# InfiniteNightmare/HNSW-Slim

Hardware: AMD Instinct MI355X
Metric: QPS @ recall@10>=0.95 (SIFT-1M d=128, k=10) (higher is better)
Workload: dtype f32

## Files before the change

### hnsw-slim_amd/csrc/flat_search.hip

```cpp
#include <hip/hip_runtime.h>

#include <algorithm>
#include <cfloat>
#include <climits>

#include "dist_recipe.hpp"
#include "engine.hpp"
#include "heap_emul.hpp"
#include "narrow_load.hpp"
#include "search_common.hpp"
#include "sorted_insert.hpp"
#include "wave_util.hpp"

namespace hs {

typedef __attribute__((address_space(3))) unsigned char lds_u8;
typedef __attribute__((address_space(3))) uint32_t lds_u32;
typedef __attribute__((address_space(3))) unsigned short lds_u16;
typedef uint32_t hs_u4 __attribute__((ext_vector_type(4)));
typedef __attribute__((address_space(3))) hs_u4 lds_u128;
typedef __attribute__((address_space(3))) float lds_f32;
typedef __attribute__((address_space(3))) hs_f2 lds_f2;
typedef unsigned short hs_us2 __attribute__((ext_vector_type(2)));

static constexpr uint32_t kFlatOvfCap = 64;
static constexpr uint32_t kFlatBucketTags = 7;

struct FlatLds { uint32_t off_q, off_vis, off_ovf, off_nid, total; };
__host__ __device__ inline FlatLds flat_layout(uint32_t dim, uint32_t ef, uint32_t nb) {
  FlatLds l;
  l.off_q = 0;
  l.off_vis = align_up(dim * 4, 16);
  const uint32_t vis_bytes = nb * 16 > (ef + 1) * 8 ? nb * 16 : (ef + 1) * 8;
  l.off_ovf = l.off_vis + align_up(vis_bytes, 16);
  l.off_nid = l.off_ovf + kFlatOvfCap * 4;
  l.total = l.off_nid + 64 * 4;
  return l;
}

__device__ __forceinline__ uint32_t pk_min_u16(uint32_t a, uint32_t b) {
  return __builtin_bit_cast(uint32_t, __builtin_elementwise_min(__builtin_bit_cast(hs_us2, a), __builtin_bit_cast(hs_us2, b)));
}
template <int METRIC>
__device__ __forceinline__ int dkey(float d) {
  const int b = (int)__float_as_uint(d);
  return METRIC == METRIC_L2 ? b : (b ^ ((b >> 31) & 0x7FFFFFFF));
}
template <int METRIC>
__device__ __forceinline__ float key_dist(int k) {
  return __uint_as_float((uint32_t)(METRIC == METRIC_L2 ? k : (k ^ ((k >> 31) & 0x7FFFFFFF))));
}
static constexpr int kFKeyInf = 0x7F800000;
static constexpr uint32_t kFDone = 0x80000000u;

__device__ __forceinline__ int wave_min_i32_f(int v) {
#define HS_SHR_MINI(ctrl) v = min(v, __builtin_amdgcn_update_dpp(INT_MAX, v, ctrl, 0xf, 0xf, false))
  HS_SHR_MINI(0x111); HS_SHR_MINI(0x112); HS_SHR_MINI(0x114); HS_SHR_MINI(0x118);
#undef HS_SHR_MINI
  const int r0 = __builtin_amdgcn_readlane(v, 15), r1 = __builtin_amdgcn_readlane(v, 31);
  const int r2 = __builtin_amdgcn_readlane(v, 47), r3 = __builtin_amdgcn_readlane(v, 63);
  return min(min(r0, r1), min(r2, r3));
}

__host__ __device__ constexpr int flat_row_buffer(int d16) {
#ifdef HS_FLAT_LONG_B
  return d16 <= 0 ? 1 : d16 <= 8 ? d16 : (d16 < HS_FLAT_LONG_B ? d16 : HS_FLAT_LONG_B);
#else
  return d16 <= 0 ? 1 : d16 <= 8 ? d16 : d16 % 30 == 0 ? 30 : d16 % 32 == 0 ? 32 : d16 % 24 == 0 ? 24 : 16;
#endif
}
__host__ __device__ constexpr int flat_waves(int s, int d16) {
#ifdef HS_FLAT_WAVES
  return HS_FLAT_WAVES;
#else
#ifdef HS_FLAT_LONG_WAVES
  return d16 > 8 ? HS_FLAT_LONG_WAVES : d16 < 0 ? 3 : s > 4 ? 4 : 5;
#else
  return d16 > 8 ? 2 : d16 < 0 ? 3 : s > 4 ? 4 : 5;
#endif
#endif
}


template <int METRIC, int D16, typename ROW>
__device__ __forceinline__ float flat_dist8(const ROW *vec, uint32_t dim, const lds_u8 *qv, uint32_t rowid, int s) {
  const lds_f2 *qq = reinterpret_cast<const lds_f2 *>(qv) + s;
  hs_f2 acc = {0.f, 0.f};
  auto step = [&](const hs_f2 q2, const hs_f2 x) {
    if (METRIC == METRIC_L2) {
      const hs_f2 t = q2 - x;
      const hs_f2 p = t * t;
      acc = acc + p;
    } else {
      acc = __builtin_elementwise_fma(q2, x, acc);
    }
  };
  if constexpr (RowKind<ROW>::narrow) {
    const ROW *chunk = vec + (size_t)rowid * dim + (uint32_t)s * (dim >> 3);
    if constexpr (D16 > 0) {
      constexpr int NDW = D16 * (int)sizeof(ROW) / 2;
      static_assert(D16 * sizeof(ROW) % 2 == 0, "a lane's chunk is a whole number of dwords");
      const uint32_t *cp = reinterpret_cast<const uint32_t *>(chunk);
      uint32_t dw[NDW];
#pragma unroll
      for (int j = 0; j + 4 <= NDW; j += 4) {
        const hs_u4_a4 v = *reinterpret_cast<const hs_u4_a4 *>(cp + j);
        dw[j] = v.x; dw[j + 1] = v.y; dw[j + 2] = v.z; dw[j + 3] = v.w;
      }
      if constexpr ((NDW & 2) != 0) {
        const hs_u2_a4 v = *reinterpret_cast<const hs_u2_a4 *>(cp + (NDW & ~3));
        dw[NDW & ~3] = v.x; dw[(NDW & ~3) + 1] = v.y;
      }
      if constexpr ((NDW & 1) != 0) dw[NDW - 1] = cp[NDW - 1];
#pragma unroll
      for (int i = 0; i < D16; i++) {
        if (D16 > 8 && i % 8 == 0) __builtin_amdgcn_sched_barrier(0);
        step(qq[i * 8], narrow_pair((const ROW *)nullptr, dw, i));
      }
    } else {
      constexpr uint32_t RB = D16 == 0 ? 8u : 16u;
      const uint32_t steps = dim >> 4;
      for (uint32_t r0 = 0; r0 < steps; r0 += RB) {
        const uint32_t nb = min(RB, steps - r0);
        hs_f2 buf[RB];
#pragma unroll
        for (uint32_t i = 0; i < RB; i++)
          if (i < nb) buf[i] = narrow_pair_at(chunk, r0 + i);
#pragma unroll
        for (uint32_t i = 0; i < RB; i++)
          if (i < nb) step(qq[(r0 + i) * 8], buf[i]);
      }
    }
  } else {
  const hs_f2 *row = reinterpret_cast<const hs_f2 *>(vec + (size_t)rowid * dim) + s;
  if (D16 > 0) {
    constexpr int B = flat_row_buffer(D16);
    constexpr int R = (D16 > 0 ? D16 : 1) / B, T = (D16 > 0 ? D16 : 1) % B;
    hs_f2 buf[B];
#pragma unroll
    for (int i = 0; i < B; i++) buf[i] = row[i * 8];
#pragma unroll
    for (int i = 0; i < B; i++) {
      if (B > 8 && i % 8 == 0) __builtin_amdgcn_sched_barrier(0);
      step(qq[i * 8], buf[i]);
    }
#pragma unroll 1
    for (int r = 1; r < R; r++) {
#pragma unroll
      for (int i = 0; i < B; i++) buf[i] = row[(r * B + i) * 8];
#pragma unroll
      for (int i = 0; i < B; i++) step(qq[(r * B + i) * 8], buf[i]);
    }
    if (T > 0) {
#pragma unroll
      for (int i = 0; i < T; i++) buf[i] = row[(R * B + i) * 8];
#pragma unroll
      for (int i = 0; i < T; i++) step(qq[(R * B + i) * 8], buf[i]);
    }
  } else {
    constexpr uint32_t RB = D16 == 0 ? 8u : 16u;
    const uint32_t steps = dim >> 4;
    for (uint32_t r0 = 0; r0 < steps; r0 += RB) {
      const uint32_t nb = min(RB, steps - r0);
      hs_f2 buf[RB];
#pragma unroll
      for (uint32_t i = 0; i < RB; i++)
        if (i < nb) buf[i] = row[(r0 + i) * 8];
#pragma unroll
      for (uint32_t i = 0; i < RB; i++)
        if (i < nb) step(qq[(r0 + i) * 8], buf[i]);
    }
  }
  }
  if (METRIC == METRIC_L2) {
    float r = acc.x + acc.y;
#pragma unroll
    for (int k = 1; k < 8; k++) {
      float t;
      asm("s_nop 1\n\tv_add_f32_dpp %0, %1, %2 row_shr:1 row_mask:0xf bank_mask:0xf" : "=v"(t) : "v"(r), "v"(acc.x));
      r = t + acc.y;
    }
    return r;
  } else {
    float hx = acc.x + dpp_f<0x104>(acc.x), hy = acc.y + dpp_f<0x104>(acc.y);
    hx = hx + dpp_f<0x102>(hx); hy = hy + dpp_f<0x102>(hy);
    hx = hx + dpp_f<0x101>(hx); hy = hy + dpp_f<0x101>(hy);
    return 1.0f - (hx + hy);
  }
}

struct FlatHeap {
  lds_u8 *lds;
  uint2 *glob;
  uint32_t L;
};
typedef uint32_t hs_u2 __attribute__((ext_vector_type(2)));
typedef __attribute__((address_space(3))) hs_u2 lds_u64;
template <bool T2>
__device__ __forceinline__ uint2 fh_get(const FlatHeap &h, uint32_t s) {
  if (!T2 || s < h.L) { const hs_u2 v = *reinterpret_cast<lds_u64 *>(h.lds + s * 8); return make_uint2(v.x, v.y); }
  return h.glob[s];
}
template <bool T2>
__device__ __forceinline__ void fh_set(const FlatHeap &h, uint32_t s, uint2 v) {
  if (!T2 || s < h.L) *reinterpret_cast<lds_u64 *>(h.lds + s * 8) = hs_u2{v.x, v.y};
  else h.glob[s] = v;
}
template <bool T2>
__device__ __forceinline__ uint4 fh_get2(const FlatHeap &h, uint32_t s ) {
  if (!T2 || s < h.L) { const hs_u4 v = *reinterpret_cast<lds_u128 *>(h.lds + s * 8); return make_uint4(v.x, v.y, v.z, v.w); }
  return *reinterpret_cast<const uint4 *>(&h.glob[s]);
}
template <bool T2>
__device__ __forceinline__ void fh_push(const FlatHeap &h, uint32_t n , float d, uint32_t id, int lane) {
  const uint32_t anc = n >> (lane + 1);
  const bool has = anc != 0 && lane < 31;
  uint2 p = make_uint2(0, 0);
  if (has) p = fh_get<T2>(h, anc);
  const unsigned long long rises = hs_ballot(has && __uint_as_float(p.x) > d);
  const uint32_t r = __ffsll((long long)~rises) - 1;
  if ((uint32_t)lane < r) fh_set<T2>(h, n >> lane, p);
  if ((uint32_t)lane == r) fh_set<T2>(h, n >> r, make_uint2(__float_as_uint(d), id));
}
template <bool T2>
__device__ __forceinline__ void fh_pop(const FlatHeap &h, uint32_t n ) {
  if (n <= 1) return;
  const uint2 v = fh_get<T2>(h, n);
  const uint32_t len = n - 1;
  uint32_t hole = 0, child = 0;
  while (child < (len - 1) / 2) {
    child = 2 * (child + 1);
    const uint4 two = fh_get2<T2>(h, child);
    const bool left = __uint_as_float(two.z) > __uint_as_float(two.x);
    fh_set<T2>(h, hole + 1, left ? make_uint2(two.x, two.y) : make_uint2(two.z, two.w));
    child = left ? child - 1 : child;
    hole = child;
  }
  if ((len & 1) == 0 && child == (len - 2) / 2) {
    child = 2 * (child + 1);
    fh_set<T2>(h, hole + 1, fh_get<T2>(h, child));
    hole = child - 1;
  }
  const float vd = __uint_as_float(v.x);
  while (hole > 0) {
    const uint32_t parent = (hole - 1) >> 1;
    const uint2 p = fh_get<T2>(h, parent + 1);
    if (!(__uint_as_float(p.x) > vd)) break;
    fh_set<T2>(h, hole + 1, p);
    hole = parent;
  }
  fh_set<T2>(h, hole + 1, v);
}

__device__ __forceinline__ void fh_pop_wave(const FlatHeap &h, uint32_t n , int lane) {
  if (n <= 1) return;
  const uint2 v = fh_get<false>(h, n);
  const uint32_t len = n - 1;
  uint32_t hole = 0;
  const uint32_t dl = lane < 1 ? 0u : (lane < 3 ? 1u : 2u);
  const uint32_t ol = (uint32_t)lane + 1u - (1u << dl);
  while (true) {
    const uint32_t node = ((hole + 1u) << dl) - 1u + ol;
    const bool two = lane < 7 && 2u * node + 2u < len;
    uint4 pr = make_uint4(0, 0, 0, 0);
    if (two) pr = fh_get2<false>(h, 2u * node + 2u);
    const bool right = !(__uint_as_float(pr.z) > __uint_as_float(pr.x));
    const unsigned long long vm = hs_ballot(two), rm = hs_ballot(two && right);
    uint32_t l = 0, path = 0, last = 0;
    bool open = true;
#pragma unroll
    for (int kk = 0; kk < 3; kk++) {
      const bool ok = open && ((vm >> l) & 1ull);
      if (ok) { path |= 1u << l; last = l; l = 2u * l + 1u + (uint32_t)((rm >> l) & 1ull); }
      open = ok;
    }
    if (path == 0) break;
    const uint32_t child = 2u * node + 1u + (right ? 1u : 0u);
    if (lane < 7 && ((path >> lane) & 1u)) fh_set<false>(h, node + 1u, right ? make_uint2(pr.z, pr.w) : make_uint2(pr.x, pr.y));
    hole = __builtin_amdgcn_readlane(child, last);
    if (!open) break;
  }
  if ((len & 1u) == 0 && hole == (len - 2u) / 2u) {
    const uint2 c = fh_get<false>(h, 2u * hole + 2u);
    if (lane == 0) fh_set<false>(h, hole + 1u, c);
    hole = 2u * hole + 1u;
  }
  wave_sync();
  fh_push<false>(h, hole + 1u, __uint_as_float(v.x), v.y, lane);
}

struct FlatSync {
  lds_u8 *vis;
  uint32_t *scratch;
  uint32_t heap_lds_slots, off_heap, off_log, off_hop, hop_cap, cand_total;
  uint32_t n_log, hop0, hl, lb_bits;
  uint32_t cand_size, hp, hq, h_idx;
};
struct FlatSyncOut { uint32_t cand_size, hp, hq, h_idx, rc, stop, next_id; };
#ifdef HS_FLAT_SYNC_CALL
#define HS_FLAT_SYNC_ATTR __attribute__((noinline))
#else
#define HS_FLAT_SYNC_ATTR __forceinline__
#endif
template <int METRIC>
__device__ HS_FLAT_SYNC_ATTR FlatSyncOut flat_heap_sync(FlatSync f) {
  const int lane = threadIdx.x;
  lds_u8 *vis = (lds_u8 *)(uintptr_t)uni((uint32_t)(uintptr_t)f.vis);
  const uint64_t sbits = (uint64_t)(uintptr_t)f.scratch;
  uint32_t *scratch = reinterpret_cast<uint32_t *>((uintptr_t)(((uint64_t)uni((uint32_t)(sbits >> 32)) << 32) | uni((uint32_t)sbits)));
  uint2 *heap_store = reinterpret_cast<uint2 *>(scratch + uni(f.off_heap));
  const uint2 *tlog = reinterpret_cast<const uint2 *>(scratch + uni(f.off_log));
  const uint32_t *hoplog = scratch + uni(f.off_hop);
  hs_u4 *park = reinterpret_cast<hs_u4 *>(scratch + uni(f.off_hop) + uni(f.hop_cap));
  const uint32_t heap_lds_slots = uni(f.heap_lds_slots), n_log = uni(f.n_log), hop0 = uni(f.hop0), hl = f.hl, cand_total = uni(f.cand_total);
  const int lb = (int)uni(f.lb_bits);
  uint32_t cand_size = uni(f.cand_size), hp = uni(f.hp), hq = uni(f.hq), h_idx = uni(f.h_idx), rc = 0, next_id = 0;
  __threadfence_block();
  for (uint32_t i = lane; i * 2u < heap_lds_slots; i += 64) park[i] = *reinterpret_cast<lds_u128 *>(vis + i * 16);
  FlatHeap cand;
  cand.lds = vis;
  cand.L = heap_lds_slots;
  cand.glob = heap_store;
  wave_sync();
  for (uint32_t sl = lane; sl <= cand_size && sl < heap_lds_slots; sl += 64) {
    const uint2 e = heap_store[sl];
    *reinterpret_cast<lds_u64 *>(vis + sl * 8) = hs_u2{e.x, e.y};
  }
  wave_sync();
  uint32_t ebase = ~0u;
  uint2 eb = make_uint2(0, 0);
  auto log_at = [&](uint32_t i) -> uint2 {
    if ((i & ~63u) != ebase) {
      ebase = i & ~63u;
      eb = (ebase + lane < n_log) ? tlog[ebase + lane] : make_uint2(0, 0);
    }
    return make_uint2(__builtin_amdgcn_readlane(eb.x, i & 63u), __builtin_amdgcn_readlane(eb.y, i & 63u));
  };
  if (h_idx == 0) {
    const uint2 e = log_at(0);
    cand_size = 1;
    fh_push<false>(cand, cand_size, __uint_as_float(e.x), e.y, lane);
    wave_sync();
    h_idx = 1;
  }
  const uint32_t ring_base = hop0 & ~63u;
  uint32_t hbase = ~0u, hcnt = 0;
  while (hq < hop0) {
    if (hp == hq) {
      if (cand_size < heap_lds_slots) fh_pop_wave(cand, cand_size, lane);
      else if (lane == 0) fh_pop<true>(cand, cand_size);
      cand_size--;
      hp++;
      wave_sync();
    }
    if ((hq & ~63u) != hbase) {
      hbase = hq & ~63u;
      hcnt = hbase == ring_base ? hl : hoplog[hbase + lane];
    }
    const uint32_t np = (uint32_t)__builtin_amdgcn_readlane(hcnt, hq & 63u);
    if (__builtin_expect(cand_size + np > cand_total, 0)) { rc = 2; break; }
    const bool in_lds = cand_size + np < heap_lds_slots;
    for (uint32_t q = 0; q < np; q++) {
      const uint2 e = log_at(h_idx);
      cand_size++;
      if (in_lds) fh_push<false>(cand, cand_size, __uint_as_float(e.x), e.y, lane);
      else fh_push<true>(cand, cand_size, __uint_as_float(e.x), e.y, lane);
      wave_sync();
      h_idx++;
    }
    hq++;
  }
  bool stop = rc != 0 || cand_size == 0;
  if (!stop) {
    const uint2 root = fh_get<false>(cand, 1);
    const uint32_t rkey_bits = uni(root.x);
    if (dkey<METRIC>(__uint_as_float(rkey_bits)) > lb) {
      stop = true;
    } else {
      next_id = uni(root.y);
      if (cand_size < heap_lds_slots) fh_pop_wave(cand, cand_size, lane);
      else if (lane == 0) fh_pop<true>(cand, cand_size);
      cand_size--;
      hp++;
      wave_sync();
    }
  }
  for (uint32_t sl = lane; sl <= cand_size && sl < heap_lds_slots; sl += 64) {
    const hs_u2 e = *reinterpret_cast<lds_u64 *>(vis + sl * 8);
    heap_store[sl] = make_uint2(e.x, e.y);
  }
  wave_sync();
  __threadfence_block();
  for (uint32_t i = lane; i * 2u < heap_lds_slots; i += 64) *reinterpret_cast<lds_u128 *>(vis + i * 16) = park[i];
  wave_sync();
  FlatSyncOut o;
  o.cand_size = cand_size; o.hp = hp; o.hq = hq; o.h_idx = h_idx; o.rc = rc; o.stop = stop ? 1u : 0u; o.next_id = next_id;
  return o;
}

template <int S>
__device__ __forceinline__ int rank_key(const int (&tk)[S], uint32_t r) {
  const uint32_t l = r / S, sl = r % S;
  int v = __builtin_amdgcn_readlane(tk[0], l);
#pragma unroll
  for (int s = 1; s < S; s++) {
    const int t = __builtin_amdgcn_readlane(tk[s], l);
    v = sl == (uint32_t)s ? t : v;
  }
  return v;
}

template <int METRIC, int S, int D16, typename ROW>
__device__ int search_one_flat(const DevIndex &ix, const SearchArgs &a, const uint32_t qi, lds_u8 *smem, const ROW *rows) {
  const int lane = threadIdx.x;
  constexpr int OWN = METRIC == METRIC_L2 ? 7 : 0;
  const int s8 = lane & 7, grp = lane >> 3;
  const uint32_t dim = D16 > 0 ? (uint32_t)D16 * 16u : ix.dim;
  const FlatLds L = flat_layout(dim, a.ef, a.fl_nb);
  lds_u8 *qv = smem + L.off_q;
  lds_u8 *vis = smem + L.off_vis;
  lds_u32 *ovf = reinterpret_cast<lds_u32 *>(smem + L.off_ovf);
  lds_u32 *nid = reinterpret_cast<lds_u32 *>(smem + L.off_nid);
  const uint32_t k = a.k, ef = a.ef;
  uint32_t *scratch = a.spill + (size_t)qi * a.spill_stride;
  uint2 *tlog = reinterpret_cast<uint2 *>(scratch + a.spill_slots + 2 * a.cand2_cap);
  uint32_t *hoplog = scratch + a.spill_slots + 2 * a.cand2_cap + 2 * a.log_cap;
  const uint32_t hop_cap = a.hop_cap / 4;
  uint32_t n_dist = 1, n_hops = 0, n_nbr = 0;
#ifdef HS_FLAT_DIAG
  const unsigned long long diag_t0 = __builtin_amdgcn_s_memrealtime();
  uint32_t diag_syncs = 0, diag_replayed = 0, diag_sync_ticks = 0, diag_pre = 0;
  uint32_t diag_ph[6] = {0, 0, 0, 0, 0, 0};
  unsigned long long diag_tp = __builtin_amdgcn_s_memtime();
#define HS_DIAG_LAP(i) { const unsigned long long t_ = __builtin_amdgcn_s_memtime(); diag_ph[i] += (uint32_t)(t_ - diag_tp); diag_tp = t_; }
#else
#define HS_DIAG_LAP(i)
#endif

  for (uint32_t i = lane; i < dim; i += 64) reinterpret_cast<lds_f32 *>(qv)[i] = a.queries[(size_t)qi * dim + i];
  for (uint32_t i = lane; i < a.fl_nb; i += 64) *reinterpret_cast<lds_u128 *>(vis + i * 16) = hs_u4{~0u, ~0u, ~0u, 0x0000FFFFu};
  uint32_t ovf_n = 0;
  const uint32_t vmask = a.vis_bits >= 32 ? 0xFFFFFFFFu : (1u << a.vis_bits) - 1u;
  const uint32_t nb = a.fl_nb, vmul = a.fl_mul, vsh = a.fl_sh;
  wave_sync();

  bool vfail = false;
  Visited v2;
  v2.t2 = scratch;
  v2.slots2 = a.spill_slots;
  v2.limit2 = a.spill_slots - (a.spill_slots >> 2);
  v2.n2 = 0;
  v2.spilled = false;
  auto vis_mark = [&](const uint32_t id, const bool valid) -> bool {
    const uint32_t h32 = id * 2654435761u;
    const uint32_t h = h32 & vmask;
    const uint32_t tag = __umulhi(h, vmul) >> vsh;
    const uint32_t b = h - tag * nb;
    lds_u8 *bp = vis + b * 16;
    const hs_u4 w = *reinterpret_cast<lds_u128 *>(bp);
    const uint32_t t2 = tag | (tag << 16);
    const uint32_t m = pk_min_u16(pk_min_u16(w.x ^ t2, w.y ^ t2), pk_min_u16(w.z ^ t2, (w.w ^ tag) | 0xFFFF0000u));
    const bool hit = (m & 0xFFFFu) == 0 || (m >> 16) == 0;
    bool isnew = valid && !hit;
    bool done = false;
    unsigned long long lm = hs_ballot(isnew && (w.w >> 16) >= kFlatBucketTags);
    if (__builtin_expect(lm != 0 && ovf_n != 0, 0)) {
      const uint32_t mine = (uint32_t)lane < ovf_n ? ovf[lane] : kNone;
      unsigned long long todo = lm;
      while (todo) {
        const int j = __ffsll((long long)todo) - 1;
        todo &= todo - 1;
        const uint32_t idj = __builtin_amdgcn_readlane(id, j);
        const bool found = hs_ballot(mine == idj) != 0;
        if (found && lane == j) isnew = false;
      }
      if (v2.spilled) {
        const bool mine2 = isnew && ((lm >> lane) & 1ull);
        if (mine2) { isnew = vis_insert_t2(v2, id, h32); done = true; }
        v2.n2 += __popcll(hs_ballot(mine2 && isnew));
      }
    }
    uint32_t e = 0;
    if (isnew && !done) {
      const uint32_t old = __hip_atomic_fetch_add(reinterpret_cast<lds_u32 *>(bp + 12), 0x10000u, __ATOMIC_RELAXED, __HIP_MEMORY_SCOPE_WAVEFRONT);
      e = old >> 16;
      if (e < kFlatBucketTags) *reinterpret_cast<lds_u16 *>(bp + e * 2) = (unsigned short)tag;
    }
    const bool over = isnew && !done && e >= kFlatBucketTags;
    const unsigned long long om = hs_ballot(over);
    if (__builtin_expect(om != 0, 0)) {
      const uint32_t at = ovf_n + __popcll(om & ((1ull << lane) - 1ull));
      const bool to_list = over && at < kFlatOvfCap;
      if (to_list) ovf[at] = id;
      const uint32_t room = kFlatOvfCap - ovf_n;
      const uint32_t want = __popcll(om);
      ovf_n += min(want, room);
      if (want > room) {
        if (!v2.spilled) {
          uint32_t i0 = lane;
          if constexpr (RowKind<ROW>::narrow) asm volatile("" : "+v"(i0));
          for (uint32_t i = i0; i < v2.slots2; i += 64) v2.t2[i] = kEmpty;
          __threadfence_block();
          v2.spilled = true;
          if (lane == 0) atomicAdd(a.counters + 3, 1u);
        }
        if (over && !to_list) vis_insert_t2(v2, id, h32);
        v2.n2 += want - room;
      }
      if (v2.n2 > v2.limit2) vfail = true;
      wave_sync();
    }
    return isnew;
  };

  uint32_t cur = ix.enterpoint;
  float curdist = 0.f;
  if (a.phase == 2) {
    const uint4 e = a.entry[qi];
    cur = uni(e.x);
    curdist = unif(__uint_as_float(e.y));
    n_dist = uni(e.z);
    n_hops = uni(e.w);
    n_nbr = n_dist - 1;
  } else {
    {
      const float d = flat_dist8<METRIC, D16>(rows, dim, qv, cur, s8);
      curdist = __uint_as_float(__builtin_amdgcn_readlane(__float_as_uint(d), OWN));
    }
    uint32_t cur_b = ix.ep_base;
    for (int lvl = ix.maxlevel; lvl > 0; lvl--) {
      bool changed = true;
      while (changed) {
        changed = false;
        n_hops++;
        if (cur_b == kNone) continue;
        uint2 pr = make_uint2(kNone, kNone);
        if ((uint32_t)lane < ix.up_stride) pr = ix.uptile[(size_t)(cur_b + lvl - 1) * ix.up_stride + lane];
        const uint32_t m = __popcll(hs_ballot(pr.x != kNone));
        if (m == 0) continue;
        n_nbr += m;
        n_dist += m;
        int best_key = INT_MAX;
        uint32_t best_at = 0;
        for (uint32_t base = 0; base < m; base += 8) {
          const uint32_t j = base + grp;
          const uint32_t rid = __shfl(pr.x, (int)(j < m ? j : base), 64);
          const float d = flat_dist8<METRIC, D16>(rows, dim, qv, rid, s8);
          const int ky = (s8 == OWN && j < m) ? dkey<METRIC>(d) : INT_MAX;
          const int mn = wave_min_i32_f(ky);
          if (mn < best_key) {
            best_key = mn;
            best_at = base + ((uint32_t)(__ffsll((long long)hs_ballot(ky == mn)) - 1) >> 3);
          }
        }
        if (best_key < dkey<METRIC>(curdist)) {
          curdist = key_dist<METRIC>(best_key);
          cur = __builtin_amdgcn_readlane(pr.x, best_at);
          cur_b = __builtin_amdgcn_readlane(pr.y, best_at);
          changed = true;
        }
      }
    }
    if (a.phase == 1) {
      if (lane == 0) a.entry[qi] = make_uint4(cur, __float_as_uint(curdist), n_dist, n_hops);
      return 0;
    }
  }
  if (ix.kind == 0) n_dist++;

  int tk[S];
  uint32_t ti[S];
  unsigned long long inr[S];
#pragma unroll
  for (int s = 0; s < S; s++) {
    tk[s] = kFKeyInf;
    ti[s] = kFDone;
    inr[s] = hs_ballot((uint32_t)(lane * S + s) < ef);
  }
  const int laneS = lane * S;
  const bool exact_fit = ef == 64u * S;
  {
    const bool mine = lane == 0 || (lane == 1 && a.mark_ep && ix.enterpoint != cur);
    vis_mark(lane == 0 ? cur : ix.enterpoint, mine);
  }
  if (lane == 0) {
    tk[0] = dkey<METRIC>(curdist);
    ti[0] = cur;
    tlog[0] = make_uint2(__float_as_uint(curdist), cur);
  }
  int lb = rank_key<S>(tk, ef - 1);
  uint32_t n_log = 1;
  uint32_t hop0 = 0;
  uint32_t hl = 0;
  int ghost_key = INT_MIN;
  bool btie = false;
  uint32_t cand_size = 0, hp = 0, hq = 0, h_idx = 0;
  const uint32_t stride = ix.tile_stride;
  int rc = vfail ? 1 : 0;

  const uint32_t lb_lane = (ef - 1) / S, lb_slot = (ef - 1) % S;
  auto bound_key = [&]() -> int {
    int v = __builtin_amdgcn_readlane(tk[0], lb_lane);
#pragma unroll
    for (int s = 1; s < S; s++) {
      const int t = __builtin_amdgcn_readlane(tk[s], lb_lane);
      v = lb_slot == (uint32_t)s ? t : v;
    }
    return v;
  };
  struct Near { bool any; int p, slot, key; uint32_t id, same; };
  auto nearest = [&]() -> Near {
    Near r;
    unsigned long long um[S], any = 0;
#pragma unroll
    for (int s = 0; s < S; s++) {
      um[s] = hs_ballot((int)ti[s] >= 0) & inr[s];
      any |= um[s];
    }
    r.any = any != 0;
    r.p = 0; r.slot = 0; r.key = kFKeyInf; r.id = 0; r.same = 0;
    if (any) {
      const int p = __ffsll((long long)any) - 1;
      int u_key = __builtin_amdgcn_readlane(tk[S - 1], p);
      uint32_t u_id = __builtin_amdgcn_readlane(ti[S - 1], p);
      int u_slot = S - 1;
#pragma unroll
      for (int s = S - 2; s >= 0; s--) {
        const bool here = (um[s] >> p) & 1ull;
        const int kk = __builtin_amdgcn_readlane(tk[s], p);
        const uint32_t ii = __builtin_amdgcn_readlane(ti[s], p);
        u_key = here ? kk : u_key;
        u_id = here ? ii : u_id;
        u_slot = here ? s : u_slot;
      }
      uint32_t same = 0;
#pragma unroll
      for (int s = 0; s < S; s++) same += __popcll(hs_ballot(tk[s] == u_key) & um[s]);
      r.p = p; r.slot = u_slot; r.key = u_key; r.id = u_id; r.same = same;
    }
    return r;
  };
  bool have_pre = false;
  uint32_t pre_id = 0, pre_tile = kNone;
  int pre_key = 0;

  while (rc == 0) {
    uint32_t next_id = 0, id = kNone;
    bool need_heap = false;
    if (have_pre && !(ghost_key == lb && pre_key == lb)) {
      next_id = pre_id;
      id = pre_tile;
    } else {
      if (have_pre) {
#pragma unroll
        for (int s = 0; s < S; s++) ti[s] = ti[s] == (pre_id | kFDone) ? pre_id : ti[s];
      }
      const Near u = nearest();
      const bool any = u.any;
      need_heap = ghost_key == lb;
      if (any) {
        need_heap = u.same > 1 || (need_heap && u.key == lb);
        next_id = u.id;
      } else if (!need_heap) {
        break;
      }
    if (__builtin_expect(need_heap, 0)) {
#ifdef HS_FLAT_DIAG
      diag_syncs += any == 0 ? 0x10000u : (ghost_key == lb ? 0x100u : 1u);
      diag_replayed += hop0 - hq;
      const unsigned long long diag_s0 = __builtin_amdgcn_s_memrealtime();
#endif
      FlatSync fs;
      fs.vis = vis; fs.heap_lds_slots = min(a.fl_nb * 2u, 1024u) & ~1u; fs.scratch = scratch; fs.off_heap = a.spill_slots;
      fs.off_log = a.spill_slots + 2 * a.cand2_cap; fs.off_hop = fs.off_log + 2 * a.log_cap; fs.hop_cap = hop_cap;
      fs.cand_total = a.cand2_cap - 2; fs.n_log = n_log; fs.hop0 = hop0; fs.hl = hl; fs.lb_bits = (uint32_t)lb;
      fs.cand_size = cand_size; fs.hp = hp; fs.hq = hq; fs.h_idx = h_idx;
      const FlatSyncOut fo = flat_heap_sync<METRIC>(fs);
      cand_size = fo.cand_size; hp = fo.hp; hq = fo.hq; h_idx = fo.h_idx;
#ifdef HS_FLAT_DIAG
      diag_sync_ticks += (uint32_t)(__builtin_amdgcn_s_memrealtime() - diag_s0);
#endif
      if (fo.rc != 0) { rc = (int)fo.rc; break; }
      if (fo.stop) break;
      next_id = fo.next_id;
    }
#pragma unroll
      for (int s = 0; s < S; s++) ti[s] = ti[s] == next_id ? (next_id | kFDone) : ti[s];
      if ((uint32_t)lane < stride) id = ix.tile0[(size_t)next_id * stride + lane];
    }
#ifdef HS_FLAT_DIAG
    diag_pre += have_pre ? 1u : 0u;
    HS_DIAG_LAP(0);
    asm volatile("s_waitcnt vmcnt(0)" ::: "memory");
    HS_DIAG_LAP(1);
#endif
    have_pre = false;
    n_hops++;
    const bool valid = id != kNone;
    const uint32_t m = __popcll(hs_ballot(valid));
    const bool isnew = vis_mark(id, valid);
    if (__builtin_expect(vfail, 0)) { rc = 1; break; }
    const unsigned long long nm = hs_ballot(isnew);
    const uint32_t cnt = __popcll(nm);
    n_nbr += m;
    n_dist += cnt;
    if (isnew) nid[__popcll(nm & ((1ull << lane) - 1ull))] = id;
    wave_sync();
    HS_DIAG_LAP(2);
    uint32_t n_acc_hop = 0;
    for (uint32_t base = 0; base < cnt; base += 8) {
      const uint32_t j = base + grp;
      const bool act = j < cnt;
      const uint32_t rid = nid[act ? j : base];
      const float d = flat_dist8<METRIC, D16>(rows, dim, qv, rid, s8);
      const int my_key = (s8 == OWN && act) ? dkey<METRIC>(d) : kFKeyInf;
#ifdef HS_FLAT_DIAG
      asm volatile("s_nop 0" : : "v"(my_key) : "memory");
      HS_DIAG_LAP(3);
#endif
      int b_lane = -1;
      if (base + 8 >= cnt && ghost_key != lb) {
        const Near u = nearest();
        int mk = min(my_key, __builtin_amdgcn_update_dpp(kFKeyInf, my_key, 0x118, 0xf, 0xf, false));
        const int b_key = min(min(__builtin_amdgcn_readlane(mk, OWN + 8), __builtin_amdgcn_readlane(mk, OWN + 24)),
                              min(__builtin_amdgcn_readlane(mk, OWN + 40), __builtin_amdgcn_readlane(mk, OWN + 56)));
        const bool b_ok = b_key < lb;
        if (b_ok && (!u.any || b_key < u.key)) {
          const unsigned long long bm = hs_ballot(my_key == b_key);
          if (__popcll(bm) == 1) {
            b_lane = __ffsll((long long)bm) - 1;
            have_pre = true;
            pre_key = b_key;
            pre_id = __builtin_amdgcn_readlane(rid, b_lane);
          }
        } else if (u.any && u.same == 1 && (!b_ok || u.key < b_key)) {
          const uint32_t below = __popcll(hs_ballot(my_key < u.key));
          if ((uint32_t)(u.p * S + u.slot) + below < ef) {
            have_pre = true;
            pre_key = u.key;
            pre_id = u.id;
#pragma unroll
            for (int s = 0; s < S; s++) ti[s] = ti[s] == pre_id ? (pre_id | kFDone) : ti[s];
          }
        }
        pre_tile = kNone;
        if (have_pre && (uint32_t)lane < stride) pre_tile = ix.tile0[(size_t)pre_id * stride + lane];
      }
      constexpr bool kRankFree = D16 <= 8;
      unsigned long long todo = hs_ballot(my_key < lb);
      unsigned long long am = 0;
      while (todo) {
        const int jl = __ffsll((long long)todo) - 1;
        todo &= todo - 1;
        const int kj = __builtin_amdgcn_readlane(my_key, jl);
        if (kj < lb) {
          const uint32_t idj = __builtin_amdgcn_readlane(rid, jl) | (jl == b_lane ? kFDone : 0u);
          am |= 1ull << jl;
          const int ek = lb;
          const uint32_t ei = __builtin_amdgcn_readlane(ti[S - 1], 63);
          const int upk = __builtin_amdgcn_update_dpp(kInsertKeyMin, tk[S - 1], 0x138, 0xf, 0xf, false);
          const uint32_t upi = (uint32_t)__builtin_amdgcn_update_dpp(0, (int)ti[S - 1], 0x138, 0xf, 0xf, false);
          if constexpr (kRankFree) {
            sorted_insert_lane<S>(tk, ti, upk, upi, kj, idj);
          } else {
            uint32_t pos = 0;
#pragma unroll
            for (int s = 0; s < S; s++) pos += __popcll(hs_ballot(tk[s] <= kj));
#pragma unroll
            for (int s = S - 1; s >= 1; s--) {
              const bool gt = (uint32_t)(laneS + s) > pos;
              tk[s] = gt ? tk[s - 1] : tk[s];
              ti[s] = gt ? ti[s - 1] : ti[s];
            }
            {
              const bool gt = (uint32_t)laneS > pos;
              tk[0] = gt ? upk : tk[0];
              ti[0] = gt ? upi : ti[0];
            }
            {
              const uint32_t pl = pos / S, ps = pos % S;
#pragma unroll
              for (int s = 0; s < S; s++)
                if (ps == (uint32_t)s) {
                  tk[s] = (int)write_lane((uint32_t)tk[s], (uint32_t)kj, pl);
                  ti[s] = write_lane(ti[s], idj, pl);
                }
            }
          }
          lb = bound_key();
          if (__builtin_expect(exact_fit, 0)) {
            if (ek != kFKeyInf && lb == ek) {
              btie = true;
              if ((int)ei >= 0) ghost_key = ek;
            }
          }
        }
      }
      if (am) {
        const uint32_t at = n_log + __popcll(am & ((1ull << lane) - 1ull));
        if (((am >> lane) & 1ull) && at < a.log_cap) tlog[at] = make_uint2(__float_as_uint(d), rid);
        const uint32_t na = __popcll(am);
        n_log += na;
        n_acc_hop += na;
      }
      HS_DIAG_LAP(4);
    }
    if (!exact_fit && n_acc_hop != 0 && lb != kFKeyInf) {
      unsigned long long eq = 0, un = 0;
#pragma unroll
      for (int s = 0; s < S; s++) {
        const unsigned long long e = hs_ballot(tk[s] == lb) & ~inr[s];
        eq |= e;
        un |= e & hs_ballot((int)ti[s] >= 0);
      }
      if (eq) btie = true;
      if (un) ghost_key = lb;
      if (__builtin_expect(rank_key<S>(tk, 64 * S - 1) == lb, 0)) { rc = 3; break; }
    }
    hl = write_lane(hl, uni(n_acc_hop), uni(hop0 & 63u));
    hop0++;
    if (__builtin_expect((hop0 & 63u) == 0, 0)) {
      if (hop0 > hop_cap) { rc = 3; break; }
      hoplog[hop0 - 64 + lane] = hl;
    }
    if (__builtin_expect(n_log > a.log_cap, 0)) { rc = 3; break; }
    HS_DIAG_LAP(5);
  }
  if (__builtin_expect(rc == 1 || rc == 2, 0)) {
    flag_query(a, qi, ST_OVERFLOW, rc - 1, lane);
    return rc;
  }
  if (__builtin_expect(rc == 3, 0)) return 3;

  const uint32_t top_size = min(n_log, ef), valid_n = min(top_size, k);
  const bool watch = ef == k;
  const bool replay = (top_size > k && rank_key<S>(tk, k - 1) == rank_key<S>(tk, k)) || (watch && btie);
  if (__builtin_expect(!replay, 1)) {
#pragma unroll
    for (int s = 0; s < S; s++) {
      const uint32_t r = laneS + s;
      if (r < k) {
        const bool v = r < valid_n;
        const uint64_t label = v ? ix.labels[ti[s] & ~kFDone] : ~0ull;
        if (a.out_labels32) a.out_labels32[(size_t)qi * k + r] = v ? (uint32_t)label : 0xFFFFFFFFu;
        if (a.out_labels64) a.out_labels64[(size_t)qi * k + r] = label;
        if (a.out_dists) a.out_dists[(size_t)qi * k + r] = v ? key_dist<METRIC>(tk[s]) : __builtin_inff();
      }
    }
  } else {
    if (lane == 0) atomicAdd(a.counters + 2, 1u);
    __threadfence_block();
    Pair *top = reinterpret_cast<Pair *>((unsigned char *)smem + L.off_vis);
    uint32_t ts = 0;
    for (uint32_t base = 0; base < n_log; base += 64) {
      const uint32_t mm = min(64u, n_log - base);
      uint2 e = make_uint2(0, 0);
      if ((uint32_t)lane < mm) e = tlog[base + lane];
      for (uint32_t j = 0; j < mm; j++) {
        const float d = __uint_as_float(__builtin_amdgcn_readlane(e.x, j));
        const uint32_t nbj = __builtin_amdgcn_readlane(e.y, j);
        if (lane == 0) {
          top[ts].d = d;
          top[ts].id = nbj;
          push_heap(top, (long)ts + 1, LessD());
          if (ts + 1 > ef) pop_heap(top, (long)ts + 1, LessD());
        }
        ts = min(ts + 1, ef);
      }
    }
    if (lane == 0) {
      if (a.mode == 0) {
        if (ts >= k) nth_element(top, (long)k, (long)ts, LessD());
      } else {
        uint32_t t2 = ts;
        while (t2 > k) { pop_heap(top, (long)t2, LessD()); t2--; }
      }
    }
    wave_sync();
    for (uint32_t i = lane; i < k; i += 64) {
      const bool v = i < valid_n;
      const Pair p = v ? top[i] : Pair{__builtin_inff(), 0};
      const uint64_t label = v ? ix.labels[p.id] : ~0ull;
      if (a.out_labels32) a.out_labels32[(size_t)qi * k + i] = v ? (uint32_t)label : 0xFFFFFFFFu;
      if (a.out_labels64) a.out_labels64[(size_t)qi * k + i] = label;
      if (a.out_dists) a.out_dists[(size_t)qi * k + i] = p.d;
    }
  }
  if (lane == 0) {
    if (a.out_counts) a.out_counts[qi] = valid_n;
    if (a.stats) {
      a.stats[qi * 4 + 0] = n_dist;
      a.stats[qi * 4 + 1] = n_hops;
      a.stats[qi * 4 + 2] = n_nbr;
      a.stats[qi * 4 + 3] = replay ? 1u : a.pass_id;
#ifdef HS_FLAT_DIAG
      uint32_t *dg = a.stats + (size_t)a.nq * 4 + qi * 16;
      dg[4] = (uint32_t)diag_t0;
      dg[5] = diag_sync_ticks;
      dg[6] = diag_pre;
      for (int i = 0; i < 6; i++) dg[8 + i] = diag_ph[i];
      dg[0] = (uint32_t)(__builtin_amdgcn_s_memrealtime() - diag_t0);
      dg[1] = diag_syncs;
      dg[2] = diag_replayed;
      dg[3] = ovf_n | (v2.spilled ? 0x10000u : 0u) | (v2.n2 << 17);
#endif
    }
    a.status[qi] = ST_DONE;
  }
  return 0;
}

#if !defined(HS_TU_ROWS) || HS_TU_ROWS == 0
#define HS_ROWS_ID f32
#define HS_KERNEL(name) name
#define HS_ROWS_PARAM
#define HS_ROWS_READ ix.vec
#define HS_ROWS_ARG
#else
#if HS_TU_ROWS == 1
#define HS_ROWS_ID u8
#define HS_KERNEL(name) name##_u8
typedef uint8_t TuRow;
#else
#define HS_ROWS_ID f16
#define HS_KERNEL(name) name##_f16
typedef _Float16 TuRow;
#endif
#define HS_ROWS_PARAM , const TuRow *rows
#define HS_ROWS_READ rows
#define HS_ROWS_ARG , reinterpret_cast<const TuRow *>(rows)
#endif
template <int METRIC, int S, int D16>
__global__ void __launch_bounds__(64) __attribute__((amdgpu_waves_per_eu(flat_waves(S, D16)))) HS_KERNEL(flat_kernel)(DevIndex ix, SearchArgs a HS_ROWS_PARAM) {
  extern __shared__ __align__(16) unsigned char smem_raw[];
  lds_u8 *smem = (lds_u8 *)smem_raw;
  for (uint32_t it = blockIdx.x; it < a.nq; it += gridDim.x) {
    const uint32_t qi = (a.phase == 2 && a.order) ? a.order[it] : it;
    if (a.pass_id != 0 && !((1u << a.status[qi]) & a.select_mask)) continue;
    const int rc = search_one_flat<METRIC, S, D16>(ix, a, qi, smem, HS_ROWS_READ);
    if (rc == 3 && threadIdx.x == 0) a.status[qi] = ST_HAZARD;
    wave_sync();
  }
}

struct FlatShape { int S, D16; };
constexpr FlatShape flat_shape(uint32_t dim, uint32_t ef) {
  return {ef <= 64 ? 1 : ef <= 128 ? 2 : ef <= 192 ? 3  : ef <= 256 ? 4 : ef <= 384 ? 6 : 8,
          dim == 128 ? 8 : dim == 96 ? 6 : dim == 960 ? 60 : dim > 256 ? -1 : 0};
}
template <int METRIC, int D16>
static hipError_t flat_launch_d(const DevIndex &ix, const SearchArgs &a, const void *rows, hipStream_t stream, int s) {
  const size_t lds = flat_layout(ix.dim, a.ef, a.fl_nb).total;
  switch (s) {
    case 1: return launch_kernel(HS_KERNEL(flat_kernel)<METRIC, 1, D16>, ix, a, lds, stream HS_ROWS_ARG);
    case 2: return launch_kernel(HS_KERNEL(flat_kernel)<METRIC, 2, D16>, ix, a, lds, stream HS_ROWS_ARG);
    case 3: return launch_kernel(HS_KERNEL(flat_kernel)<METRIC, 3, D16>, ix, a, lds, stream HS_ROWS_ARG);
    case 4: return launch_kernel(HS_KERNEL(flat_kernel)<METRIC, 4, D16>, ix, a, lds, stream HS_ROWS_ARG);
    case 6: return launch_kernel(HS_KERNEL(flat_kernel)<METRIC, 6, D16>, ix, a, lds, stream HS_ROWS_ARG);
    default: return launch_kernel(HS_KERNEL(flat_kernel)<METRIC, 8, D16>, ix, a, lds, stream HS_ROWS_ARG);
  }
}
template <int METRIC>
static hipError_t flat_launch_s(const DevIndex &ix, const SearchArgs &a, const void *rows, hipStream_t stream) {
  const FlatShape sh = flat_shape(ix.dim, a.ef);
  switch (sh.D16) {
    case 8: return flat_launch_d<METRIC, 8>(ix, a, rows, stream, sh.S);
    case 6: return flat_launch_d<METRIC, 6>(ix, a, rows, stream, sh.S);
    case 60: return flat_launch_d<METRIC, 60>(ix, a, rows, stream, sh.S);
    case -1: return flat_launch_d<METRIC, -1>(ix, a, rows, stream, sh.S);
    default: return flat_launch_d<METRIC, 0>(ix, a, rows, stream, sh.S);
  }
}

#if !defined(HS_TU_ROWS) || HS_TU_ROWS == 0
#if !defined(HS_TU_METRIC) || HS_TU_METRIC == 0
__global__ void __launch_bounds__(64) flat_heap_ops_kernel(const uint32_t *ops, uint32_t n_ops, uint2 *spill, uint2 *out_heap, uint2 *out_pops,
                                                            uint32_t *out_n, int wave_pop, uint32_t lds_slots) {
  extern __shared__ __align__(16) unsigned char smem_raw[];
  const int lane = threadIdx.x;
  FlatHeap h;
  h.lds = (lds_u8 *)smem_raw;
  h.L = lds_slots;
  h.glob = spill;
  uint32_t size = 0, pops = 0;
  for (uint32_t i = 0; i < n_ops; i++) {
    const uint32_t kind = uni(ops[3 * i]), key = uni(ops[3 * i + 1]), id = uni(ops[3 * i + 2]);
    if (kind == 0) {
      size++;
      if (size < h.L) fh_push<false>(h, size, __uint_as_float(key), id, lane);
      else fh_push<true>(h, size, __uint_as_float(key), id, lane);
    } else if (size > 0) {
      const uint2 root = fh_get<true>(h, 1);
      if (lane == 0) out_pops[pops] = root;
      pops++;
      if (wave_pop && size < h.L) fh_pop_wave(h, size, lane);
      else if (lane == 0) { if (size < h.L) fh_pop<false>(h, size); else fh_pop<true>(h, size); }
      size--;
    }
    wave_sync();
  }
  for (uint32_t s = lane; s < size; s += 64) out_heap[s] = fh_get<true>(h, s + 1);
  if (lane == 0) { out_n[0] = size; out_n[1] = pops; }
}
hipError_t flat_heap_ops(const uint32_t *d_ops, uint32_t n_ops, uint2 *d_spill, uint2 *d_heap, uint2 *d_pops, uint32_t *d_n, int wave_pop,
                         uint32_t lds_slots, hipStream_t stream) {
  hipLaunchKernelGGL(flat_heap_ops_kernel, dim3(1), dim3(64), (size_t)lds_slots * 8, stream, d_ops, n_ops, d_spill, d_heap, d_pops, d_n, wave_pop, lds_slots);
  return hipGetLastError();
}
#endif

#if !defined(HS_TU_METRIC) || HS_TU_METRIC == 0
bool flatk_supported(const DevIndex &ix, uint32_t ef, uint32_t k) {
  return ix.tile0 != nullptr && (ix.maxlevel == 0 || ix.uptile != nullptr) && ix.threshold_level == 0 && !ix.has_deleted && ix.n > 0 &&
         ix.n < kFDone && (ix.dim & 15u) == 0 && ef >= k && ef <= 512 && k <= 64;
}
uint32_t flatk_waves_per_cu(uint32_t dim, uint32_t ef) {
  const FlatShape sh = flat_shape(dim, ef);
  return 4u * (uint32_t)flat_waves(sh.S, sh.D16);
}
size_t flatk_lds_bytes(uint32_t dim, uint32_t ef, uint32_t nb) { return flat_layout(dim, ef, nb).total; }
#endif
#endif

#if !defined(HS_TU_METRIC) || HS_TU_METRIC == 0
hipError_t HS_LAUNCHER(flat, HS_ROWS_ID, l2)(const DevIndex &ix, const SearchArgs &a, const void *rows, hipStream_t stream, const FilterArgs *) {
  return flat_launch_s<METRIC_L2>(ix, a, rows, stream);
}
#endif
#if !defined(HS_TU_METRIC) || HS_TU_METRIC == 1
hipError_t HS_LAUNCHER(flat, HS_ROWS_ID, ip)(const DevIndex &ix, const SearchArgs &a, const void *rows, hipStream_t stream, const FilterArgs *) {
  return flat_launch_s<METRIC_IP>(ix, a, rows, stream);
}
#endif

}
```

Measured before the change: 15.03 million.

## Software-pipeline neighbor row loads ahead of distance compute in flat search

Splits the f32 distance routine into a load-issue phase and a finish phase, so the next batch of neighbor rows can be fetched into registers while the current batch's distances are reduced. Both the upper-level greedy descent and the base-layer expansion loop get this, and a per-configuration hop-order table picks which variant is used. For some variants the nearest-candidate scan is moved ahead of the distance finish, and an evicted-slot readlane is skipped unless exact_fit is set. This aims to hide global memory latency at the cost of extra row-buffer registers, which may lower occupancy.

Result: no change. 15.17 million (median of 6 runs) (+1.0%).

```diff
diff --git a/hnsw-slim_amd/csrc/flat_search.hip b/hnsw-slim_amd/csrc/flat_search.hip
--- a/hnsw-slim_amd/csrc/flat_search.hip
+++ b/hnsw-slim_amd/csrc/flat_search.hip
@@ -81,20 +81,76 @@
 #endif
 }
 
+__host__ __device__ constexpr int flat_hop_order(int metric, int s, int d16) {
+#ifdef HS_FLAT_HOP_ORDER
+  return HS_FLAT_HOP_ORDER;
+#else
+  switch (metric * 1000 + s * 100 + d16) {
+    case 206: case 306: case 308: case 806: case 1206: case 1306: case 1806: return 3;
+    case 106: case 208: case 1308: return 7;
+    case 1406: return 1;
+    default: return 0;
+  }
+#endif
+}
+
+
+template <int METRIC>
+__device__ __forceinline__ void flat_step(hs_f2 &acc, const hs_f2 q2, const hs_f2 x) {
+  if (METRIC == METRIC_L2) {
+    const hs_f2 t = q2 - x;
+    const hs_f2 p = t * t;
+    acc = acc + p;
+  } else {
+    acc = __builtin_elementwise_fma(q2, x, acc);
+  }
+}
+template <int METRIC>
+__device__ __forceinline__ float flat_lane_sum(const hs_f2 acc) {
+  if (METRIC == METRIC_L2) {
+    float r = acc.x + acc.y;
+#pragma unroll
+    for (int k = 1; k < 8; k++) {
+      float t;
+      asm("s_nop 1\n\tv_add_f32_dpp %0, %1, %2 row_shr:1 row_mask:0xf bank_mask:0xf" : "=v"(t) : "v"(r), "v"(acc.x));
+      r = t + acc.y;
+    }
+    return r;
+  } else {
+    float hx = acc.x + dpp_f<0x104>(acc.x), hy = acc.y + dpp_f<0x104>(acc.y);
+    hx = hx + dpp_f<0x102>(hx); hy = hy + dpp_f<0x102>(hy);
+    hx = hx + dpp_f<0x101>(hx); hy = hy + dpp_f<0x101>(hy);
+    return 1.0f - (hx + hy);
+  }
+}
+
+template <int D16>
+constexpr bool flat_rows_split(bool narrow) { return !narrow && D16 >= 1 && D16 <= 8; }
+template <int D16>
+__device__ __forceinline__ void flat_rows_issue(hs_f2 (&buf)[D16], const float *vec, uint32_t rowid, int s) {
+  const hs_f2 *row = reinterpret_cast<const hs_f2 *>(vec + (size_t)rowid * ((uint32_t)D16 * 16u)) + s;
+#pragma unroll
+  for (int i = 0; i < D16; i++) buf[i] = row[i * 8];
+}
+template <int METRIC, int D16>
+__device__ __forceinline__ float flat_rows_finish(const hs_f2 (&buf)[D16], const lds_u8 *qv, int s) {
+  const lds_f2 *qq = reinterpret_cast<const lds_f2 *>(qv) + s;
+  hs_f2 acc = {0.f, 0.f};
+#pragma unroll
+  for (int i = 0; i < D16; i++) flat_step<METRIC>(acc, qq[i * 8], buf[i]);
+  return flat_lane_sum<METRIC>(acc);
+}
 
 template <int METRIC, int D16, typename ROW>
 __device__ __forceinline__ float flat_dist8(const ROW *vec, uint32_t dim, const lds_u8 *qv, uint32_t rowid, int s) {
+  if constexpr (flat_rows_split<D16>(RowKind<ROW>::narrow)) {
+    hs_f2 buf[D16];
+    flat_rows_issue<D16>(buf, vec, rowid, s);
+    return flat_rows_finish<METRIC, D16>(buf, qv, s);
+  } else {
   const lds_f2 *qq = reinterpret_cast<const lds_f2 *>(qv) + s;
   hs_f2 acc = {0.f, 0.f};
-  auto step = [&](const hs_f2 q2, const hs_f2 x) {
-    if (METRIC == METRIC_L2) {
-      const hs_f2 t = q2 - x;
-      const hs_f2 p = t * t;
-      acc = acc + p;
-    } else {
-      acc = __builtin_elementwise_fma(q2, x, acc);
-    }
-  };
+  auto step = [&](const hs_f2 q2, const hs_f2 x) { flat_step<METRIC>(acc, q2, x); };
   if constexpr (RowKind<ROW>::narrow) {
     const ROW *chunk = vec + (size_t)rowid * dim + (uint32_t)s * (dim >> 3);
     if constexpr (D16 > 0) {
@@ -172,20 +228,7 @@
     }
   }
   }
-  if (METRIC == METRIC_L2) {
-    float r = acc.x + acc.y;
-#pragma unroll
-    for (int k = 1; k < 8; k++) {
-      float t;
-      asm("s_nop 1\n\tv_add_f32_dpp %0, %1, %2 row_shr:1 row_mask:0xf bank_mask:0xf" : "=v"(t) : "v"(r), "v"(acc.x));
-      r = t + acc.y;
-    }
-    return r;
-  } else {
-    float hx = acc.x + dpp_f<0x104>(acc.x), hy = acc.y + dpp_f<0x104>(acc.y);
-    hx = hx + dpp_f<0x102>(hx); hy = hy + dpp_f<0x102>(hy);
-    hx = hx + dpp_f<0x101>(hx); hy = hy + dpp_f<0x101>(hy);
-    return 1.0f - (hx + hy);
+  return flat_lane_sum<METRIC>(acc);
   }
 }
 
@@ -414,6 +457,9 @@
 __device__ int search_one_flat(const DevIndex &ix, const SearchArgs &a, const uint32_t qi, lds_u8 *smem, const ROW *rows) {
   const int lane = threadIdx.x;
   constexpr int OWN = METRIC == METRIC_L2 ? 7 : 0;
+  constexpr int kHopOrder = flat_rows_split<D16>(RowKind<ROW>::narrow) ? flat_hop_order(METRIC, S, D16) : 0;
+  constexpr bool kSplit = kHopOrder != 0;
+  constexpr int kRowBuf = kSplit ? D16 : 1;
   const int s8 = lane & 7, grp = lane >> 3;
   const uint32_t dim = D16 > 0 ? (uint32_t)D16 * 16u : ix.dim;
   const FlatLds L = flat_layout(dim, a.ef, a.fl_nb);
@@ -542,10 +588,19 @@
         n_dist += m;
         int best_key = INT_MAX;
         uint32_t best_at = 0;
+        constexpr bool kUpSplit = (kHopOrder & 4) != 0;
+        hs_f2 ubuf[kUpSplit ? kRowBuf : 1];
+        if constexpr (kUpSplit) flat_rows_issue<D16>(ubuf, rows, __shfl(pr.x, (int)((uint32_t)grp < m ? grp : 0), 64), s8);
         for (uint32_t base = 0; base < m; base += 8) {
           const uint32_t j = base + grp;
-          const uint32_t rid = __shfl(pr.x, (int)(j < m ? j : base), 64);
-          const float d = flat_dist8<METRIC, D16>(rows, dim, qv, rid, s8);
+          float d;
+          if constexpr (kUpSplit) {
+            d = flat_rows_finish<METRIC, D16>(ubuf, qv, s8);
+            if (base + 8 < m) flat_rows_issue<D16>(ubuf, rows, __shfl(pr.x, (int)(j + 8 < m ? j + 8 : base + 8), 64), s8);
+          } else {
+            const uint32_t rid = __shfl(pr.x, (int)(j < m ? j : base), 64);
+            d = flat_dist8<METRIC, D16>(rows, dim, qv, rid, s8);
+          }
           const int ky = (s8 == OWN && j < m) ? dkey<METRIC>(d) : INT_MAX;
           const int mn = wave_min_i32_f(ky);
           if (mn < best_key) {
@@ -708,11 +763,40 @@
     wave_sync();
     HS_DIAG_LAP(2);
     uint32_t n_acc_hop = 0;
+    hs_f2 rbuf[kRowBuf];
+    uint32_t rid_ahead = 0;
+    if constexpr (kSplit) {
+      if (cnt != 0) {
+        rid_ahead = nid[(uint32_t)grp < cnt ? grp : 0];
+        flat_rows_issue<D16>(rbuf, rows, rid_ahead, s8);
+      }
+    }
     for (uint32_t base = 0; base < cnt; base += 8) {
       const uint32_t j = base + grp;
       const bool act = j < cnt;
-      const uint32_t rid = nid[act ? j : base];
-      const float d = flat_dist8<METRIC, D16>(rows, dim, qv, rid, s8);
+      Near u = {false, 0, 0, kFKeyInf, 0, 0};
+      uint32_t rid;
+      float d;
+      if constexpr (kSplit) {
+        if (!(kHopOrder & 2) && base != 0) {
+          rid_ahead = nid[act ? j : base];
+          flat_rows_issue<D16>(rbuf, rows, rid_ahead, s8);
+        }
+        rid = rid_ahead;
+        if (kHopOrder & 1) {
+          const bool pre = base + 8 >= cnt && ghost_key != lb;
+          if (pre) u = nearest();
+          __builtin_amdgcn_sched_barrier(0);
+        }
+        d = flat_rows_finish<METRIC, D16>(rbuf, qv, s8);
+        if ((kHopOrder & 2) && base + 8 < cnt) {
+          rid_ahead = nid[j + 8 < cnt ? j + 8 : base + 8];
+          flat_rows_issue<D16>(rbuf, rows, rid_ahead, s8);
+        }
+      } else {
+        rid = nid[act ? j : base];
+        d = flat_dist8<METRIC, D16>(rows, dim, qv, rid, s8);
+      }
       const int my_key = (s8 == OWN && act) ? dkey<METRIC>(d) : kFKeyInf;
 #ifdef HS_FLAT_DIAG
       asm volatile("s_nop 0" : : "v"(my_key) : "memory");
@@ -720,7 +804,7 @@
 #endif
       int b_lane = -1;
       if (base + 8 >= cnt && ghost_key != lb) {
-        const Near u = nearest();
+        if (!(kSplit && (kHopOrder & 1))) u = nearest();
         int mk = min(my_key, __builtin_amdgcn_update_dpp(kFKeyInf, my_key, 0x118, 0xf, 0xf, false));
         const int b_key = min(min(__builtin_amdgcn_readlane(mk, OWN + 8), __builtin_amdgcn_readlane(mk, OWN + 24)),
                               min(__builtin_amdgcn_readlane(mk, OWN + 40), __builtin_amdgcn_readlane(mk, OWN + 56)));
@@ -757,7 +841,8 @@
           const uint32_t idj = __builtin_amdgcn_readlane(rid, jl) | (jl == b_lane ? kFDone : 0u);
           am |= 1ull << jl;
           const int ek = lb;
-          const uint32_t ei = __builtin_amdgcn_readlane(ti[S - 1], 63);
+          uint32_t ei = kFDone;
+          if (!kSplit || __builtin_expect(exact_fit, 0)) ei = __builtin_amdgcn_readlane(ti[S - 1], 63);
           const int upk = __builtin_amdgcn_update_dpp(kInsertKeyMin, tk[S - 1], 0x138, 0xf, 0xf, false);
           const uint32_t upi = (uint32_t)__builtin_amdgcn_update_dpp(0, (int)ti[S - 1], 0x138, 0xf, 0xf, false);
           if constexpr (kRankFree) {
```
